# nv-tlabs/ASE

Measured on AMD Instinct MI355X. Metric: ASE PPO-update samples/sec (4096 envs x horizon 32), higher is better.
Workload: dtype f16; 1 GPU; BASELINE configs[1]: ASE agent, 4096 envs x horizon 32, obs 253 / act 31 / amp obs 1400 / latent 64, [1024,1024,512] MLPs + disc + shared-trunk encoder, minibatch 16384 (amp 4096) x 6 mini-epochs = 48 optimisation steps per update; random-init weights; precision_choice=auto without an oracle leg: the first candidate, replay=program, parallelism=single GPU

## Files before the change

### ase_amd/csrc/gemm.hip

```cpp
#include "gemm_nt.h"
#include <math.h>

namespace ase_nt {

unsigned long long* g_nt_prof = nullptr;
int g_nt_prof_clk = 0;

int nt_choice(int M, int N, int K, int es, bool b16) {
    if (N <= 64) return 0;
    const int t256 = ((M + 255) / 256) * ((N + 255) / 256);
    const bool big = N % 256 == 0 && t256 >= 192 && (t256 <= 256 || t256 % 256 == 0 || t256 >= 1024);
    if (big) {
        if (!(b16 && (K * es) % 128 == 0)) return 3;
        const int t192 = ((M + 191) / 192) * (N / 256);
        return (t256 < 256 && t192 <= 256 && t192 > t256) ? 6 : 2;
    }
    if ((K * es) % 128 != 0) return 1;
    const int t128 = ((M + 127) / 128) * ((N + 127) / 128), t64x128 = ((M + 63) / 64) * ((N + 127) / 128);
    if (t128 >= 512) return 1;
    if (t64x128 >= 512) return 4;
    return 5;
}

}

using namespace ase_nt;

extern "C" int ase_hip_debug_nt_profile(void* buf) {
    g_nt_prof = reinterpret_cast<unsigned long long*>(buf);
    return ASE_OK;
}

extern "C" int ase_hip_debug_nt_profile_clock(int shader_clock) {
    g_nt_prof_clk = shader_clock ? 1 : 0;
    return ASE_OK;
}

extern "C" int ase_hip_gemm_nt_kernel_id(int M, int N, int K, int dtype) {
    dtype &= 0xFF;
    return nt_choice(M, N, K, ase_elem_size(dtype), ase_elem_size(dtype) == 2);
}

namespace {

struct NTFused {
    const float* seed_w = nullptr; int seed_n = 0; float seed_scale = 0.f;
    void* twin = nullptr; int64_t ldtwin = 0; int twin_dtype = 0;
    double* sq_acc = nullptr; double sq_scale = 0.0; const float* sq_dyn = nullptr;
    bool any() const { return seed_w || twin || sq_acc; }
};

int gemm_nt_impl(const void* A, int64_t lda, const void* B, int64_t ldb, void* C, int64_t ldc,
                 const float* bias, const void* aux, int64_t ldaux, int aux_split, int aux_delta,
                 float* colsum, int colsum_n, void* mask_out, int64_t ldmask, int M, int N, int K, int act,
                 int aux_mode, int out_f32, float alpha, float* alpha_dev, int dtype_word, const NTFused& fu, void* stream) {
    const int dtype = dtype_word & 0xFF, ea = (dtype_word >> 8) & 0xFF, eb = (dtype_word >> 16) & 0xFF;
    const int es = ase_elem_size(dtype);
    ASE_CHECK_ARG(dtype == ASE_F32 || dtype == ASE_BF16 || dtype == ASE_F32X3 || dtype == ASE_F16 || dtype == ASE_F32H3,
                  "gemm_nt: bad dtype %d", dtype);
    ASE_CHECK_ARG(ea >= 0 && ea <= 24 && eb >= 0 && eb <= 24 && (dtype == ASE_F32H3 || (ea | eb) == 0),
                  "gemm_nt: operand scale exponents (bits 8-15 / 16-23 of dtype) are 0..24 and belong to ASE_F32H3 only");
    ASE_CHECK_ARG(A && B && (C || fu.twin) && M > 0 && N > 0 && K > 0, "gemm_nt: null/empty operand (M=%d N=%d K=%d)", M, N, K);
    if (fu.any()) {
        ASE_CHECK_ARG(dtype == ASE_F32H3 && colsum == nullptr && act <= ASE_ACT_RELU &&
                          (aux_mode == ASE_AUX_NONE || aux_mode == ASE_AUX_RELU_BITS),
                      "gemm_nt_ex: seed / twin / sum of squares belong to ASE_F32H3 launches without column sums, with no activation or "
                      "ReLU and no mask operand or a bit matrix");
        ASE_CHECK_ARG(fu.seed_w == nullptr || (fu.seed_n >= 0 && fu.seed_n <= N), "gemm_nt_ex: seed_n=%d outside [0, N]", fu.seed_n);
        ASE_CHECK_ARG(fu.twin == nullptr || ((fu.twin_dtype == ASE_F16 || fu.twin_dtype == ASE_BF16) && fu.ldtwin >= N &&
                                             ((uintptr_t)fu.twin % 8) == 0 && (fu.ldtwin * 2) % 8 == 0),
                      "gemm_nt_ex: the twin is f16 / bf16, 8-byte aligned, ldtwin >= N in whole 8-byte steps");
        ASE_CHECK_ARG(fu.sq_acc == nullptr || ((uintptr_t)fu.sq_acc % 8) == 0, "gemm_nt_ex: misaligned sq_acc");
    }
    ASE_CHECK_ARG((K * es) % 64 == 0, "gemm_nt: K=%d is not a multiple of %d elements", K, 64 / es);
    ASE_CHECK_ARG(lda >= K && ldb >= K && (ldc >= N || C == nullptr), "gemm_nt: leading dimension too small");
    ASE_CHECK_ARG(((uintptr_t)A % 16) == 0 && ((uintptr_t)B % 16) == 0 && (lda * es) % 16 == 0 && (ldb * es) % 16 == 0,
                  "gemm_nt: A/B must be 16-byte aligned with 16-byte row pitch");
    ASE_CHECK_ARG(aux_mode == ASE_AUX_NONE || aux != nullptr, "gemm_nt: aux_mode %d without aux", aux_mode);
    const bool bits = aux_mode == ASE_AUX_RELU_BITS;
    ASE_CHECK_ARG(N % 4 == 0 && ((uintptr_t)C % 16) == 0 && (ldc * (out_f32 ? 4 : es)) % 8 == 0 &&
                      (aux == nullptr || bits || (((uintptr_t)aux % 8) == 0 && (ldaux * es) % 8 == 0)),
                  "gemm_nt: C / aux must allow 8/16-byte row-vector access (N %% 4 == 0, aligned pitches)");
    ASE_CHECK_ARG(!bits || (((uintptr_t)aux % 4) == 0 && ldaux * 32 >= N), "gemm_nt: bit mask needs ldaux >= N / 32 words");
    const bool smooth = act >= ASE_ACT_SILU;
    ASE_CHECK_ARG(act >= ASE_ACT_NONE && act <= ASE_ACT_SOFTPLUS, "gemm_nt: unknown activation %d", act);
    ASE_CHECK_ARG((aux_mode & 0xFF) <= ASE_AUX_PREACT && ((aux_mode & 0xFF) == ASE_AUX_PREACT || (aux_mode >> 8) == 0) &&
                      (aux_mode >> 8) <= ASE_ACT_SOFTPLUS, "gemm_nt: bad aux_mode 0x%x", aux_mode);
// ... 54 lines not shown
```

### ase_amd/csrc/gemm_nt.h

```cpp
#pragma once
#include "common.h"
#include "act.h"
#include <type_traits>

namespace ase_nt {


__device__ __forceinline__ int xcd_remap(int bid, int nwg) {
    const int q = nwg >> 3, r = nwg & 7, xcd = bid & 7, loc = bid >> 3;
    const int base = (xcd < r) ? xcd * (q + 1) : r * (q + 1) + (xcd - r) * q;
    return base + loc;
}


template <int RB> __device__ __forceinline__ int lds_swz(int r) { return RB == 128 ? ((r >> 1) & 7) : ((r >> 2) & 3); }

typedef __attribute__((address_space(1))) const void gptr_t;
typedef __attribute__((address_space(3))) void lptr_t;

template <int N> __device__ __forceinline__ void wait_vmcnt() { asm volatile("s_waitcnt vmcnt(%0)" ::"n"(N) : "memory"); }

struct NTParams {
    const char* A; int64_t lda;
    const char* B; int64_t ldb;
// ... 70 lines not shown
template <> __device__ __forceinline__ uint32_t cvt_relu_pk16<bf16_t>(f32x2 v, float lo) {
    const f32x2 l = {lo, lo};
    return __builtin_bit_cast(uint32_t, __builtin_convertvector(__builtin_elementwise_maximum(v, l), bf16x2));
}
template <> __device__ __forceinline__ uint32_t cvt_relu_pk16<f16_t>(f32x2 v, float lo) {
    const f16_t l16 = (f16_t)__builtin_amdgcn_fmed3f(lo, -65504.f, 65504.f);
    const f16x2 hi = {(f16_t)65504.f, (f16_t)65504.f}, l = {l16, l16};
    const f16x2 c = __builtin_elementwise_maximum(__builtin_elementwise_minimum(__builtin_convertvector(v, f16x2), hi), l);
    return __builtin_bit_cast(uint32_t, c);
}

__device__ __forceinline__ uint32_t ovf_fold(uint32_t run, uint32_t packed) {
    const uint32_t mag = packed & 0x7FFF7FFFu;
    asm("v_pk_max_u16 %0, %0, %1" : "+v"(run) : "v"(mag));
    return run;
}
template <typename T> __device__ __forceinline__ bool ovf_hit(uint32_t run) {
    return (run & 0xFFFFu) >= ovf_threshold<T>() || (run >> 16) >= ovf_threshold<T>();
}

template <typename T, int AUXK, bool MASK>
__device__ __forceinline__ uint32_t rows_frag(const f32x16& c, const f32x4 (&bias)[4], uint32_t w, f32x2 al, float relu_lo, int h,
                                              uint32_t (&pk)[4][2]) {
    uint32_t mlo = 0, mhi = 0;
#pragma unroll
    for (int g = 0; g < 4; ++g)
#pragma unroll
        for (int pr = 0; pr < 2; ++pr) {
            f32x2 v = {c[g * 4 + 2 * pr], c[g * 4 + 2 * pr + 1]};
            const f32x2 b = {bias[g][2 * pr], bias[g][2 * pr + 1]};
            v = v * al + b;
            if constexpr (AUXK == 2) {
                const i32x2 keep = {(int)__builtin_amdgcn_sbfe(w, 8 * g + 2 * pr, 1), (int)__builtin_amdgcn_sbfe(w, 8 * g + 2 * pr + 1, 1)};
                v = __builtin_bit_cast(f32x2, __builtin_bit_cast(i32x2, v) & keep);
            }
            pk[g][pr] = cvt_relu_pk16<T>(v, relu_lo);
            if constexpr (MASK) {
                constexpr uint32_t INF = std::is_same<T, f16_t>::value ? 0x7C007C00u : 0x7F807F80u;
                const u16x2 one = {1, 1};
                const uint32_t d = __builtin_bit_cast(uint32_t, __builtin_bit_cast(u16x2, pk[g][pr]) - one);
                uint32_t tw;
                asm("v_pk_sub_u16 %0, %1, %2 clamp" : "=v"(tw) : "s"(INF), "v"(d));
                asm("v_pk_min_u16 %0, %0, %1" : "+v"(tw) : "s"(0x00010001u));
                const u16x2 t = __builtin_bit_cast(u16x2, tw);
                const u16x2 sh = {(unsigned short)((g & 1) * 8 + 2 * pr), (unsigned short)((g & 1) * 8 + 2 * pr + 1)};
                const uint32_t m = __builtin_bit_cast(uint32_t, t << sh);
                if (g < 2) mlo |= m; else mhi |= m;
            }
        }
    if constexpr (MASK) return ((((mlo | (mlo >> 16)) & 0xFFFFu) | ((mhi | (mhi >> 16)) << 16))) << (4 * h);
    else return 0u;
}

template <typename T, int AUXK, bool MASK, int NJ, int NI>
__device__ __forceinline__ void nt8_epilogue_rows_impl(const NTParams& p, f32x16 (&acc)[NI][NJ], int lane, int mrow0, int ncol0,
                                                       const uint32_t (&bits)[NI][NJ]) {
    const int r = lane & 31, h = lane >> 5;
    const f32x2 al = {p.alpha, p.alpha};
    const float relu_lo = (p.act == ASE_ACT_RELU) ? 0.f : -__builtin_inff();
    uint32_t ovf = 0;
    f32x4 bias[NJ][4];
#pragma unroll
    for (int j = 0; j < NJ; ++j)
#pragma unroll
        for (int g = 0; g < 4; ++g) {
            if (p.bias) bias[j][g] = *reinterpret_cast<const f32x4*>(p.bias + ncol0 + j * 32 + 8 * g + 4 * h);
            else bias[j][g] = f32x4{0.f, 0.f, 0.f, 0.f};
        }
#pragma unroll
    for (int i = 0; i < NI; ++i) {
        const int m = mrow0 + i * 32 + r;
        const bool row_ok = m < p.M;
        char* crow = p.C + (int64_t)m * p.ldc + (int64_t)ncol0 * 2 + h * 16;
        uint32_t mword[NJ];
        uint4 out[NJ][2];
#pragma unroll
        for (int j = 0; j < NJ; ++j) {
            uint32_t pk[4][2];
            mword[j] = rows_frag<T, AUXK, MASK>(acc[i][j], bias[j], AUXK == 2 ? bits[i][j] >> (4 * h) : 0u, al, relu_lo, h, pk);
#pragma unroll
            for (int g = 0; g < 4; g += 2) {
                const auto s0 = __builtin_amdgcn_permlane32_swap(pk[g][0], pk[g + 1][0], false, false);
                const auto s1 = __builtin_amdgcn_permlane32_swap(pk[g][1], pk[g + 1][1], false, false);
                out[j][g >> 1] = make_uint4(s0[0], s1[0], s0[1], s1[1]);
                ovf = ovf_fold(ovf_fold(ovf_fold(ovf_fold(ovf, s0[0]), s1[0]), s0[1]), s1[1]);
            }
        }
        if (row_ok) {
#pragma unroll
            for (int j = 0; j < NJ; ++j)
#pragma unroll
                for (int g = 0; g < 4; g += 2) *reinterpret_cast<uint4*>(crow + (j * 32 + 8 * g) * 2) = out[j][g >> 1];
        }
        if constexpr (MASK) {
#pragma unroll
            for (int jp = 0; jp < NJ; jp += 2) {
                const auto w = __builtin_amdgcn_permlane32_swap(mword[jp], mword[jp + 1], false, false);
                const uint32_t full = w[0] | w[1];
                if (row_ok) p.mask_out[(int64_t)m * p.ldmask + (ncol0 >> 5) + jp + h] = full;
            }
        }
    }
    ovf_report(p.alpha_dev, ovf_hit<T>(ovf));
}

template <typename T, int AUXK, int NJ = 2, int NI = 4>
__device__ __forceinline__ void nt8_epilogue_rows(const NTParams& p, f32x16 (&acc)[NI][NJ], int lane, int mrow0, int ncol0,
                                                  const uint32_t (&bits)[NI][NJ]) {
    if (ncol0 >= p.N) return;
    if (p.mask_out) nt8_epilogue_rows_impl<T, AUXK, true, NJ, NI>(p, acc, lane, mrow0, ncol0, bits);
    else nt8_epilogue_rows_impl<T, AUXK, false, NJ, NI>(p, acc, lane, mrow0, ncol0, bits);
}


template <int UNITS> __device__ __forceinline__ void wait_dma_units() { wait_vmcnt<2 * UNITS>(); }
__device__ __forceinline__ void wait_dma_units_rt(int units) {
    if (units >= 4) wait_vmcnt<8>();
    else if (units == 3) wait_vmcnt<6>();
    else if (units == 2) wait_vmcnt<4>();
    else if (units == 1) wait_vmcnt<2>();
    else wait_vmcnt<0>();
}
__device__ __forceinline__ void nt8_sync_in() {
    NT8_BARRIER();
    asm volatile("s_waitcnt lgkmcnt(0)" ::: "memory");
    __builtin_amdgcn_sched_barrier(0);
    __builtin_amdgcn_s_setprio(1);
}
__device__ __forceinline__ void nt8_sync_out() {
    __builtin_amdgcn_s_setprio(0);
    NT8_BARRIER();
}

#define NT_PROF_STAMP(prof, tid, slot, shader_clk)                                                              \
    do {                                                                                                        \
        if ((prof) && (tid) == 0) (prof)[slot] = (shader_clk) ? (unsigned long long)clock64() : wall_clock64(); \
    } while (0)
#define NT_PROF_CLOSE(prof, tid, slot)                         \
    do {                                                       \
        if (prof) {                                            \
            asm volatile("s_waitcnt vmcnt(0)" ::: "memory");   \
            __syncthreads();                                   \
            if ((tid) == 0) (prof)[slot] = wall_clock64();     \
        }                                                      \
    } while (0)

extern unsigned long long* g_nt_prof;
extern int g_nt_prof_clk;

int nt_choice(int M, int N, int K, int es, bool b16);

int dispatch_nt_bf16(const NTParams& p, hipStream_t s);
int dispatch_nt_f16(const NTParams& p, hipStream_t s);
int dispatch_nt_f32(const NTParams& p, hipStream_t s);
int dispatch_nt_x3(const NTParams& p, hipStream_t s);
int dispatch_nt_h3(const NTParams& p, hipStream_t s);

}
```

### ase_amd/csrc/gemm_nt_kernels.h

```cpp
#pragma once
#include "gemm_nt.h"
#include <stdlib.h>
#include <utility>

namespace {

using namespace ase_nt;

typedef uint32_t u32x4 __attribute__((ext_vector_type(4)));
template <int N, typename F, int... I> __device__ __forceinline__ void static_for_impl(F&& f, std::integer_sequence<int, I...>) {
    (f(std::integral_constant<int, I>{}), ...);
}
template <int N, typename F> __device__ __forceinline__ void static_for(F&& f) { static_for_impl<N>(f, std::make_integer_sequence<int, N>{}); }

template <typename T> struct Mma;

template <typename T> struct Mma16 {
    typedef typename V16<T>::x8 x8;
    template <int FM, int FN, int RB, bool SW = false>
    static __device__ __forceinline__ void tile(const char* sA, const char* sB, int lane, f32x16 (&acc)[FM][FN]) {
        const int r = lane & 31, h = lane >> 5, sw = lds_swz<RB>(r);
#pragma unroll
        for (int ks = 0; ks < RB / 32; ++ks) {
            x8 a[FM], b[FN];
// ... 650 lines not shown
#pragma unroll
    for (int ks = 0; ks < 4; ++ks) f[ks] = *reinterpret_cast<const i32x4*>(base + L.roff[ks]);
}

template <typename T, int KIND, bool SW, int NA = 2>
__device__ __forceinline__ void nt8_mma_issue(f32x16& c0, f32x16& c1, const i32x4 (&a0)[4], const i32x4 (&a1)[4],
                                              const i32x4 (&b)[4], const NT8Lane& L, int tile, bool live) {
#pragma unroll
    for (int ks = 0; ks < 4; ++ks) {
        if (ks == 3) NT8_BARRIER();
        c0 = nt8_mfma<T, SW>(a0[ks], b[ks], c0);
        if constexpr (NA == 2) c1 = nt8_mfma<T, SW>(a1[ks], b[ks], c1);
        if (ks == 0 || ks == 2) {
            __builtin_amdgcn_sched_barrier(0);
            if (live) nt8_piece<KIND>(L, ks >> 1, tile);
            __builtin_amdgcn_sched_barrier(0);
        }
    }
    __builtin_amdgcn_sched_barrier(0);
    __builtin_amdgcn_s_setprio(0);
    __builtin_amdgcn_sched_barrier(0);
}

template <typename T, bool TAIL, bool SW, int NI = 4>
__device__ __forceinline__ void nt8_ktile(int t, int nk, const NT8Lane& L, const char* aP, const char* bP,
                                          f32x16 (&acc)[NI][2], i32x4 (&a0)[4], i32x4 (&a1)[4], i32x4 (&b0)[4],
                                          i32x4 (&b1)[4]) {
    constexpr int RB = 128;
    const int U = 4 * nk;
    const bool l1 = !TAIL || t + 1 < nk, l2 = !TAIL || t + 2 < nk;
    nt8_read(b0, bP, L);
    nt8_read(a0, aP, L);
    nt8_read(a1, aP + 32 * RB, L);
    if (!TAIL) wait_dma_units<3>();
    else wait_dma_units_rt(min(U, 4 * t + 6) - (4 * t + 3));
    nt8_sync_in();
    nt8_mma_issue<T, 2, SW>(acc[0][0], acc[1][0], a0, a1, b0, L, t + 1, l1);
    nt8_read(b1, bP + 32 * RB, L);
    if (!TAIL) wait_dma_units<3>();
    else wait_dma_units_rt(min(U, 4 * t + 7) - (4 * t + 4));
    nt8_sync_in();
    nt8_mma_issue<T, 3, SW>(acc[0][1], acc[1][1], a0, a1, b1, L, t + 1, l1);
    nt8_read(a0, aP + 64 * RB, L);
    if constexpr (NI == 4) nt8_read(a1, aP + 96 * RB, L);
    nt8_sync_in();
    nt8_mma_issue<T, 0, SW, NI - 2>(acc[2][1], acc[NI - 1][1], a0, a1, b1, L, t + 2, l2);
    if (!TAIL) wait_dma_units<3>();
    else if (t + 1 < nk) wait_dma_units_rt(min(U, 4 * t + 9) - (4 * t + 6));
    nt8_sync_in();
    nt8_mma_issue<T, 1, SW, NI - 2>(acc[2][0], acc[NI - 1][0], a0, a1, b0, L, t + 2, l2);
}


template <typename T, bool SW, int BM = 256>
__global__ __launch_bounds__(512) void gemm_nt8_kernel(NTParams p) {
    static_assert(sizeof(T) == 2, "the phased kernel takes the 16-bit storage types");
    static_assert(BM == 256 || (BM == 192 && SW), "192-row tiles come with the row-per-lane epilogue");
    constexpr int RB = 128, BN = 256, BK = 64, WM = BM / 2, NI = WM / 32;
    constexpr int kBuf = 512 * RB;
    extern __shared__ __attribute__((aligned(16))) char smem[];
    if (p.alpha_dev) p.alpha *= *p.alpha_dev;

    const int tid = threadIdx.x, lane = tid & 63;
    const int wid = __builtin_amdgcn_readfirstlane(tid >> 6);
    const int wr = wid >> 2, wc = wid & 3;
    const int nwg = p.tiles_m * p.tiles_n;
    const int tile = xcd_remap(blockIdx.x, nwg);
    const int bm0 = (tile / p.tiles_n) * BM, bn0 = (tile % p.tiles_n) * BN;

    NT_PROF_STAMP(p.prof, tid, blockIdx.x * 4 + 0, false);
    NT8Lane L;
    {
        const int lr = lane >> 3, slot = lane & 7;
#pragma unroll
        for (int g = 0; g < 2; ++g) {
            const int ra = g * WM + wid * 8;
            const int rb = (g * 2 + (wid >> 2)) * 64 + (wid & 3) * 8;
            const int ra1 = BM == 256 ? ra + 64 : (wid >> 2) * WM + 64 + (wid & 3) * 8;
            const int rows[4] = {ra, rb, rb + 32, ra1};
#pragma unroll
            for (int kind = 0; kind < 4; ++kind) {
                const int r = rows[kind] + lr;
                const bool isB = (kind == 1 || kind == 2);
                const int64_t grow = isB ? min(bn0 + r, p.N - 1) : min(bm0 + r, p.M - 1);
                L.voff[kind][g] = (uint32_t)(grow * (isB ? p.ldb : p.lda)) + (uint32_t)((slot ^ lds_swz<RB>(r)) << 4);
                L.dst[kind][g] = (uint32_t)(uintptr_t)smem + (isB ? BM * RB : 0) + rows[kind] * RB;
            }
        }
        const int r = lane & 31, h = lane >> 5, sw = lds_swz<RB>(r);
#pragma unroll
        for (int ks = 0; ks < 4; ++ks) L.roff[ks] = r * RB + (((ks * 2 + h) ^ sw) << 4);
        L.rsA = raw_buffer(p.A);
        L.rsB = raw_buffer(p.B);
    }

    f32x16 acc[NI][2];
#pragma unroll
    for (int i = 0; i < NI; ++i)
#pragma unroll
        for (int j = 0; j < 2; ++j)
#pragma unroll
            for (int e = 0; e < 16; ++e) acc[i][j][e] = 0.f;

    AuxReg<T, 2> pre_bits[16];
    uint32_t row_bits[NI][2];
    if constexpr (!SW) {
        if (p.aux_mode == ASE_AUX_RELU_BITS) nt_aux_load<T, 4, 2, 2, 2, 2>(p, 0, lane, bm0 + wr * WM, bn0 + wc * 64, pre_bits);
    }

    const int nk = p.K / BK;
    nt8_issue<0>(L, 0);
    nt8_issue<1>(L, 0);
    nt8_issue<2>(L, 0);
    nt8_issue<3>(L, 0);
    if (nk > 1) {
        nt8_issue<0>(L, 1);
        nt8_issue<1>(L, 1);
    }
    bool mask_dma = false;
    if constexpr (SW) {
        mask_dma = p.aux_mode == ASE_AUX_RELU_BITS && bn0 + wc * 64 < p.N;
        if (mask_dma) {
            char* mlds = smem + 2 * kBuf + wid * 1024;
#pragma unroll
            for (int i = 0; i < NI; ++i) {
                const int m = bm0 + wr * WM + i * 32 + (lane & 31);
                const int ma = (m >= p.aux_split) ? m - p.aux_delta : m;
                const uint32_t* w = reinterpret_cast<const uint32_t*>(p.aux + (int64_t)min(ma, p.M - 1) * p.ldaux) +
                                    ((bn0 + wc * 64) >> 5) + (lane >> 5);
                __builtin_amdgcn_global_load_lds((gptr_t*)w, (lptr_t*)(mlds + i * 256), 4, 0, 0);
            }
        }
    }
    if (nk > 1) {
        if (mask_dma) wait_vmcnt<8 + NI>(); else wait_dma_units<4>();
    } else {
        if (mask_dma) wait_vmcnt<4 + NI>(); else wait_dma_units<2>();
    }
    NT8_BARRIER();
    NT_PROF_STAMP(p.prof, tid, blockIdx.x * 4 + 1, p.prof_clk);
    if (wr == 1) NT8_BARRIER();

    i32x4 a0[4], a1[4], b0[4], b1[4];
    const int aoff = wr * WM * RB, boff = BM * RB + wc * 64 * RB;
    int t = 0;
    for (; t + 2 < nk; ++t) {
        const char* buf = smem + (t & 1) * kBuf;
        nt8_ktile<T, false, SW, NI>(t, nk, L, buf + aoff, buf + boff, acc, a0, a1, b0, b1);
    }
    for (; t < nk; ++t) {
        const char* buf = smem + (t & 1) * kBuf;
        nt8_ktile<T, true, SW, NI>(t, nk, L, buf + aoff, buf + boff, acc, a0, a1, b0, b1);
    }
    if (wr == 0) NT8_BARRIER();
    __syncthreads();
    NT_PROF_STAMP(p.prof, tid, blockIdx.x * 4 + 2, p.prof_clk);

    float* slab = reinterpret_cast<float*>(smem) + wid * (64 * 64);
    if constexpr (SW) {
        if (p.aux_mode == ASE_AUX_RELU_BITS) {
            const uint32_t* mw = reinterpret_cast<const uint32_t*>(smem + 2 * kBuf + wid * 1024);
#pragma unroll
            for (int i = 0; i < NI; ++i) {
                row_bits[i][0] = mw[i * 64 + (lane & 31)];
                row_bits[i][1] = mw[i * 64 + 32 + (lane & 31)];
            }
            nt8_epilogue_rows<T, 2, 2, NI>(p, acc, lane, bm0 + wr * WM, bn0 + wc * 64, row_bits);
        } else nt8_epilogue_rows<T, 0, 2, NI>(p, acc, lane, bm0 + wr * WM, bn0 + wc * 64, row_bits);
    } else if constexpr (BM == 256) {
        if (p.aux_mode == ASE_AUX_RELU_BITS)
            nt_epilogue_impl<T, 4, 2, 2, 2, 2, true>(p, acc, slab, lane, bm0 + wr * 128, bn0 + wc * 64, &pre_bits);
        else
            nt_epilogue<T, 4, 2, 2, 2>(p, acc, slab, lane, bm0 + wr * 128, bn0 + wc * 64);
    }
    NT_PROF_CLOSE(p.prof, tid, blockIdx.x * 4 + 3);
}

template <typename T, bool SW = false, int BM = 256> int launch_nt8(const NTParams& p0, hipStream_t stream) {
    constexpr int lds = 2 * 512 * 128 + (SW ? 8 * 1024 : 0);
    constexpr auto kern = gemm_nt8_kernel<T, SW, BM>;
    if (const int rc = ase_dynamic_lds<kern>("gemm_nt8", lds)) return rc;
    NTParams p = p0;
    p.prof = g_nt_prof;
    p.prof_clk = g_nt_prof_clk;
    p.tiles_m = (p.M + BM - 1) / BM;
    p.tiles_n = (p.N + 255) / 256;
    ASE_LAUNCH(kern, dim3(p.tiles_m * p.tiles_n), dim3(512), lds, stream, p);
    ASE_CHECK_LAUNCH("gemm_nt8");
    return ASE_OK;
}

}
#include "gemm_nt4.h"
namespace {

inline bool rows_epi(const NTParams& p, int wave_cols) {
    return !p.out_f32 && p.N % wave_cols == 0 && p.colsum == nullptr && p.act <= ASE_ACT_RELU &&
           (p.mask_out == nullptr || p.act == ASE_ACT_RELU) &&
           (p.aux_mode == ASE_AUX_NONE || p.aux_mode == ASE_AUX_RELU_BITS);
}

template <typename T> int dispatch_nt(const NTParams& p, hipStream_t s) {
    const bool k128 = (p.K * (int)sizeof(T)) % 128 == 0;
    const bool fits32 = (int64_t)p.M * p.lda < (int64_t)0x7FFFFFFF && (int64_t)p.N * p.ldb < (int64_t)0x7FFFFFFF;
    int choice = nt_choice(p.M, p.N, p.K, (int)sizeof(T), sizeof(T) == 2);
    if ((choice == 2 || choice == 6) && !fits32) choice = 3;
    if constexpr (std::is_same<T, f32h_t>::value) {
        if (p.seed_w || p.twin || p.sq_acc) {
            switch (choice) {
                case 0: return launch_nt<T, 2, 2, 1, 1, 64, 4, 1, false, true>(p, s);
                case 2: case 3: case 6:
                    if (k128) return launch_nt<T, 4, 2, 2, 4, 128, 2, 1, false, true>(p, s);
                    return launch_nt<T, 4, 2, 2, 4, 64, 4, 1, false, true>(p, s);
                case 4: return launch_nt<T, 2, 2, 1, 2, 128, 2, 2, false, true>(p, s);
                case 5: return launch_nt<T, 2, 2, 1, 1, 128, 4, 2, false, true>(p, s);
                default:
                    if (k128) return launch_nt<T, 2, 2, 2, 2, 128, 2, 2, false, true>(p, s);
                    return launch_nt<T, 2, 2, 2, 2, 64, 4, 2, false, true>(p, s);
            }
        }
    }
    switch (choice) {
        case 0: return launch_nt<T, 2, 2, 1, 1, 64, 4>(p, s);
        case 6:
            if constexpr (sizeof(T) == 2) if (rows_epi(p, 64)) return launch_nt8<T, true, 192>(p, s);
            [[fallthrough]];
        case 2:
            if constexpr (sizeof(T) == 2) {
                if (p.M >= 65536 && rows_epi(p, 128)) return launch_nt4<T>(p, s);
                if (rows_epi(p, 64)) return launch_nt8<T, true>(p, s);
                return launch_nt8<T, false>(p, s);
            }
            [[fallthrough]];
        case 3:
            if (k128) return launch_nt<T, 4, 2, 2, 4, 128, 2>(p, s);
            return launch_nt<T, 4, 2, 2, 4, 64, 4>(p, s);
        case 4:
            if constexpr (sizeof(T) == 2) if (rows_epi(p, 64)) return launch_nt<T, 2, 2, 1, 2, 128, 2, 2, true>(p, s);
            return launch_nt<T, 2, 2, 1, 2, 128, 2, 2>(p, s);
        case 5:
            if constexpr (sizeof(T) == 2) if (rows_epi(p, 32)) return launch_nt<T, 2, 2, 1, 1, 128, 4, 2, true>(p, s);
            return launch_nt<T, 2, 2, 1, 1, 128, 4, 2>(p, s);
        default:
            if constexpr (sizeof(T) == 2) if (k128 && rows_epi(p, 64)) return launch_nt<T, 2, 2, 2, 2, 128, 2, 1, true>(p, s);
            if (k128) return launch_nt<T, 2, 2, 2, 2, 128, 2>(p, s);
            return launch_nt<T, 2, 2, 2, 2, 64, 4>(p, s);
    }
}

}
```

### ase_amd/lib.py

```python
import ctypes as C
import os

_HERE = os.path.dirname(os.path.abspath(__file__))
LIB_PATH = os.path.join(_HERE, "csrc", "libase_hip.so")

ABI_VERSION = 9
PPO_SCRATCH = 1024 * 72 + 8
PPO_SCRATCH_LS = 1024 * 136 + 8
LS_FROZEN, LS_VECTOR, LS_ROWS = 0, 1, 2
TN_SLAB = 65536 + 256
F32, BF16, F32X3, F16, F32H3 = 0, 1, 2, 3, 4
ACT_NONE, ACT_RELU, ACT_TANH, ACT_SILU, ACT_ELU, ACT_GELU, ACT_SIGMOID, ACT_SELU, ACT_SOFTPLUS = range(9)
AUX_NONE, AUX_RELU_MASK, AUX_TANH_GRAD, AUX_RELU_BITS, AUX_PREACT = 0, 1, 2, 3, 4
TASK_HEADING, TASK_LOCATION, TASK_REACH, TASK_STRIKE = range(4)
TASK_OBS_COLS = (5, 2, 3, 15)
TASK_RESET_DRAWS = (3, 2, 3, 4)
RESET_FRAME, RESET_TABLE, RESET_MOTION = range(3)
RESET_HAS_TABLE, RESET_HAS_MOTION = 1, 2
KIND_U8, KIND_I32, KIND_I64, KIND_F32 = range(4)
ROLLOUT_STORE_MAX_FIELDS, ROLLOUT_STORE_ROWS = 16, 8
INIT_DEFAULT, INIT_START, INIT_RANDOM, INIT_HYBRID = range(4)

(ACC_MASK_SUM, ACC_A_LOSS, ACC_B_LOSS, ACC_ENTROPY, ACC_CLIPPED, ACC_C_LOSS, ACC_KL, ACC_DIV, ACC_BCE_AGENT,
 ACC_BCE_DEMO, ACC_AGENT_ACC, ACC_DEMO_ACC, ACC_GP, ACC_ENC, ACC_ENC_GP, ACC_LOGIT_W2, ACC_DISC_W2, ACC_ENC_W2,
# ... 2 lines not shown
(RES_A_LOSS, RES_C_LOSS, RES_B_LOSS, RES_ENTROPY, RES_CLIP_FRAC, RES_KL, RES_DISC_LOSS, RES_DISC_GP,
 RES_DISC_LOGIT_LOSS, RES_DISC_AGENT_ACC, RES_DISC_DEMO_ACC, RES_ENC_LOSS, RES_DIV_LOSS, RES_LOSS,
 RES_MASK_SUM, RES_ENC_GP, RES_LR) = range(17)
RES_COUNT = 20

_p, _i, _i64, _f, _d = C.c_void_p, C.c_int, C.c_int64, C.c_float, C.c_double

SIGNATURES = {
    "ase_hip_gemm_nt": [_p, _i64, _p, _i64, _p, _i64, _p, _p, _i64, _i, _i, _p, _i, _p, _i64, _i, _i, _i, _i, _i, _i, _f, _p, _i, _p],
    "ase_hip_gemm_nt_ex": [_p, _i64, _p, _i64, _p, _i64, _p, _p, _i64, _i, _i, _p, _i, _p, _i64, _i, _i, _i, _i, _i, _i, _f, _p, _i,
                           _p, _i, _f, _p, _i64, _i, _p, _d, _p, _p],
    "ase_hip_gemm_tn": [_p, _i64, _p, _i64, _p, _p, _i, _i, _i, _i, _i, _i, _i, _i, _f, _p, _i, _p],
    "ase_hip_refresh_shadow": [_p, _i, _i, _p, _i64, _p, _i64, _i, _i, _i, _p],
    "ase_hip_refresh_shadow_multi": [_p, _i, _i, _p],
    "ase_hip_gather_multi": [_p, _i, _p, _i, _i, _i, _p],
    "ase_hip_rms_moments": [_p, _i64, _i, _p, _i, _i, _i, _p, _p, _p],
    "ase_hip_rms_finalize": [_p, _i, _p, _p, _i, _p, _p, _p],
    "ase_hip_rms_normalize": [_p, _i64, _i, _p, _i, _i, _i, _p, _p, _p, _i64, _p, _i64, _p, _i64, _i, _p],
    "ase_hip_rms_unnormalize": [_p, _p, _p, _i64, _p],
    "ase_hip_gather_rows": [_p, _i64, _i, _p, _i, _i, _i, _p, _i64, _i, _p],
    "ase_hip_reduce_sum": [_p, _i64, _i, _p, _i, _p],
    "ase_hip_ppo_head": [_p, _i64, _p, _i64] + [_p] * 11 + [_p, _i64, _p, _i64, _p, _p, _p, _p, _p] + [_i] * 8 + [_f] * 6 + [_p]
                        + [_i, _i64, _p, _i64, _p, _f] + [_i, _p],
    "ase_hip_disc_head": [_p, _i64, _p, _i64, _p, _p, _i, _i, _f, _f, _p, _i, _p],
    "ase_hip_enc_head": [_p, _i64, _p, _i64, _p, _i64, _p, _p, _p, _i, _i, _i, _f, _f, _p, _i, _p],
    "ase_hip_gp_seed": [_p, _i64, _p, _p, _i64, _i, _i, _f, _i, _i, _p],
    "ase_hip_gp_second": [_p, _i64, _p, _i64, _p, _i64, _p, _i64, _i, _i, _i, _i, _p],
    "ase_hip_colsum": [_p, _i64, _i, _i, _f, _p, _p],
    "ase_hip_sqnorm": [_p, _i64, _i, _i, _p, _i, _d, _p, _i, _p],
    "ase_hip_finalize_scalars": [_p, _p, _i, _i, _i, _i, _i, _i] + [_f] * 11 + [_p, _f, _p],
    "ase_hip_enc_gp_seed": [_p, _i64, _p, _i64, _p, _i64, _i, _i, _f, _i, _p],
    "ase_hip_enc_gp_back": [_p, _i64, _p, _i64, _p, _i64, _p, _i64, _p, _i, _i, _f, _p, _i, _p],
    "ase_hip_clip_scale": [_p, _i64, _p, _f, _p],
    "ase_hip_begin_step": [_p, _p, _i, _p, _i, _p, _p],
    "ase_hip_adam": [_p, _p, _p, _p, _i64, _p, _p],
    "ase_hip_axpy": [_p, _p, _i64, _f, _p],
    "ase_hip_scaler_check": [_p, _i64, _i, _p, _p],
    "ase_hip_scaler_check_multi": [_p, _i, _i, _p, _p],
    "ase_hip_scaler_fold": [_p, _p, _p],
    "ase_hip_scaler_step": [_p, _p, _p, _p, _i64, _p, _p],
    "ase_hip_disc_reward": [_p, _i64, _p, _i64, _f, _p],
    "ase_hip_enc_reward": [_p, _i64, _p, _i64, _p, _i64, _i, _f, _p],
    "ase_hip_gae": [_p, _p, _p, _p, _p, _p, _f, _f, _f, _d, _d, _p, _p, _i, _i, _p],
    "ase_hip_adv_norm": [_p, _p, _p, _p, _p, _i64, _i, _i, _p],
    "ase_hip_ring_store": [_p, _i64, _i, _p, _i, _i, _i, _p, _i64, _i64, _p],
    "ase_hip_sample_latents": [_p, _i, _i, _p, _i64, _i, _p, _i64, _i, _p],
    "ase_hip_rms_moments_multi": [_p, _p, _p, _p, _p, _p, _i, _i, _i, _p, _p],
    "ase_hip_rms_normalize_multi": [_p, _p, _p, _p, _p, _p, _p, _p, _p, _i, _i, _i, _i, _p],
    "ase_hip_rms_normalize_multi_v2": [_p, _p, _p, _p, _p, _p, _p, _p, _p, _p, _p, _i, _i, _i, _i, _p],
    "ase_hip_normalize_rows": [_p, _i64, _p, _i64, _i, _i, _p],
    "ase_hip_sample_actions": [_p, _i64, _p, _i64, _p, _p, _p, _p, _p, _p, _p, _i, _i, _i, _p],
    "ase_hip_debug_nt_profile": [_p],
    "ase_hip_debug_nt_profile_clock": [_i],
    "ase_hip_motion_state": [_p] * 6 + [_i] + [_p] * 6 + [_i, _p, _p, _i, _p, _i] + [_p] * 8,
    "ase_hip_build_amp_obs": [_p, _p, _p, _p, _p, _p, _p, _i, _i, _i, _p, _i, _i, _i, _p, _i, _i, _p],
    "ase_hip_humanoid_obs_max": [_p, _p, _p, _p, _i, _i, _i, _i, _p, _i, _p, _i64, _i, _p],
    "ase_hip_humanoid_reset": [_p, _p, _p, _p, _p, _i, _p, _p, _i, _i, _i, _f, _i, _p, _p, _p],
    "ase_hip_task_obs": [_i, _p, _p, _p, _p, _p, _i, _p, _i, _p, _i64, _i, _p],
    "ase_hip_task_reward": [_i, _p, _p, _p, _p, _p, _f, _p, _p, _i, _i, _f, _i, _p, _p],
    "ase_hip_task_reset": [_i, _p, _i, _p, _p, _p, _i, _p, _p, _i64, _i64, _p, _i64, _p, _p, _p, _p, _i64] + [_d] * 8 + [_i, _i, _p],
    "ase_hip_latent_renew": [_p, _i, _p, _i64, _p, _p, _i, _p, _i, _p, _i, _i64, _i64, _p, _i64, _p, _i64, _i, _i, _i, _p],
    "ase_hip_amp_reset": [_p] * 6 + [_i] + [_p] * 6 + [_i, _p, _i] + [_p] * 5 + [_i, _i, _p, _p, _p, _i, _p, _i64, _p, _p, _i64, _i,
                          _p, _p, _p, _p, _i, _i, _i, _f, _p, _i, _p],
    "ase_hip_amp_reset_due": [_p] * 6 + [_i] + [_p] * 6 + [_i, _p, _i] + [_p, _i] + [_p, _p, _p, _i] + [_i, _d, _i, _d, _d, _i]
                             + [_p, _i] + [_p] * 4 + [_p] * 5 + [_p, _i64, _p, _p, _i64, _i] + [_p] * 4 + [_i, _i, _i, _f, _p, _i, _p],
    "ase_hip_amp_demo_fetch": [_p] * 6 + [_i] + [_p] * 4 + [_i, _p, _p, _i, _p, _i] + [_p] * 4 + [_i, _p, _p] + [_i, _i, _f, _f, _i, _i]
                              + [_p, _i64, _i, _i, _p, _p],
    "ase_hip_rollout_store": [_p, _i, _p, _f, _f, _p, _i64, _p, _i, _p, _i64, _p, _p, _i, _p, _i64, _p, _p, _p, _i, _p, _i64, _p,
                              _i, _i, _p, _i, _p],
    "ase_hip_hrl_latent": [_p, _i64, _p, _i64, _p, _i64, _i, _i, _i, _p],
    "ase_hip_hrl_llc_action": [_p, _i64, _p, _p, _p, _i64, _i, _i, _i, _p],
    "ase_hip_hrl_accum": [_p, _p, _i, _p, _i, _p, _i64, _f, _p, _i64, _i, _i, _i, _p, _p, _p, _p, _i, _p],
    "ase_hip_clip_frames": [_p] * 6 + [_i] + [_p] * 4 + [_i, _i, _p, _p, _i] + [_p] * 7,
    "ase_hip_gemm_nt_kernel_id": [_i, _i, _i, _i],
    "ase_hip_gemm_tn_kernel_id": [_i, _i, _i, _i, _i, _i64, _i64, _i],
    "ase_hip_apply_multi": [_p, _i, _p, _p, _i, _p],
    "ase_hip_apply_multi_v2": [_p, _i, _p, _p, _p, _i, _p],
    "ase_hip_gemm_tn_grouped_plan": [_p, _i, _i, _p, _i, _p, _p, _i, _p],
    "ase_hip_prog_create": [_p],
    "ase_hip_prog_destroy": [_p],
    "ase_hip_prog_begin": [_p],
    "ase_hip_prog_end": [_p],
    "ase_hip_prog_size": [_p],
    "ase_hip_prog_launch": [_p],
    "ase_hip_prog_host": [_p, _p],
    "ase_hip_mark": [_p, _p],
    "ase_hip_wait": [_p, _i],
    "ase_hip_memset": [_p, _i, _i64, _p],
    "ase_hip_memcpy": [_p, _p, _i64, _p],
    "ase_hip_gemm_tn_grouped": [_p, _p, _i, _p, _i, _p, _p, _i, _p],
}


class AseHipError(RuntimeError):
    pass


def rollout_store_ws(n_envs):
    return 3 * ((int(n_envs) + ROLLOUT_STORE_ROWS - 1) // ROLLOUT_STORE_ROWS)


def load():
    import torch
    if not os.path.exists(LIB_PATH):
        raise AseHipError(
            f"{LIB_PATH} is missing: build it with `python -c 'import __graft_entry__ as g; g.build()'` "
# ... 27 lines not shown
```

### include/ase_hip.h

```cpp
#ifndef ASE_HIP_H
#define ASE_HIP_H

#include <stdint.h>

#ifdef __cplusplus
extern "C" {
#endif

#define ASE_HIP_ABI_VERSION 9

enum { ASE_F32 = 0, ASE_BF16 = 1, ASE_F32X3 = 2 ,
       ASE_F32H3 = 4 ,
       ASE_F16 = 3  };
enum { ASE_ACT_NONE = 0, ASE_ACT_RELU = 1, ASE_ACT_TANH = 2, ASE_ACT_SILU = 3, ASE_ACT_ELU = 4, ASE_ACT_GELU = 5,
       ASE_ACT_SIGMOID = 6, ASE_ACT_SELU = 7, ASE_ACT_SOFTPLUS = 8 };
enum { ASE_AUX_NONE = 0, ASE_AUX_RELU_MASK = 1, ASE_AUX_TANH_GRAD = 2, ASE_AUX_RELU_BITS = 3 ,
       ASE_AUX_PREACT = 4  };
enum { ASE_OK = 0, ASE_EINVAL = -1, ASE_ELAUNCH = -2, ASE_EUNSUPPORTED = -3 };

int ase_hip_abi_version(void);
const char* ase_hip_last_error(void);

int ase_hip_gemm_nt_kernel_id(int M, int N, int K, int dtype);

int ase_hip_debug_nt_profile(void* buf);
int ase_hip_debug_nt_profile_clock(int shader_clock);


int ase_hip_gemm_nt(const void* A, int64_t lda, const void* B, int64_t ldb, void* C, int64_t ldc,
                    const float* bias, const void* aux, int64_t ldaux, int aux_split, int aux_delta,
                    float* colsum, int colsum_n, void* mask_out, int64_t ldmask, int M, int N, int K, int act,
                    int aux_mode, int out_f32, float alpha, float* alpha_dev, int dtype, void* stream);

int ase_hip_gemm_nt_ex(const void* A, int64_t lda, const void* B, int64_t ldb, void* C, int64_t ldc,
                       const float* bias, const void* aux, int64_t ldaux, int aux_split, int aux_delta,
                       float* colsum, int colsum_n, void* mask_out, int64_t ldmask, int M, int N, int K, int act,
                       int aux_mode, int out_f32, float alpha, float* alpha_dev, int dtype,
                       const float* seed_w, int seed_n, float seed_scale, void* twin, int64_t ldtwin, int twin_dtype,
                       double* sq_acc, double sq_scale, const float* sq_dyn, void* stream);

int ase_hip_gemm_tn(const void* A, int64_t lda, const void* B, int64_t ldb, float* G, float* gbias,
                    int bias_rows, int M, int N, int K, int n_real, int k_real, int split_src, int split_dst,
                    float alpha, const float* alpha_dev, int dtype, void* stream);

int ase_hip_gemm_tn_kernel_id(int M, int N, int K, int n_real, int bias_rows, int64_t lda, int64_t ldb, int dtype);

#define ASE_TN_SLAB (65536 + 256)
int ase_hip_gemm_tn_grouped_plan(int64_t* problems, int n_problems, int target_wg, int32_t* work, int max_work,
                                 int* n_work, int32_t* red, int max_red, int* n_red);
int ase_hip_gemm_tn_grouped(const int64_t* problems, const int32_t* work, int n_work, const int32_t* red, int n_red,
                            float* workspace, const float* alpha_dev, int dtype, void* stream);

int ase_hip_refresh_shadow(const float* W, int n_real, int k_real, void* Ws, int64_t ldws,
                           void* Wts, int64_t ldwts, int split_src, int split_dst, int dtype,
                           void* stream);

int ase_hip_refresh_shadow_multi(const int64_t* desc, int n_layers, int dtype, void* stream);


int ase_hip_rms_moments(const float* src, int64_t ld_src, int D, const int32_t* idx, int remap_h,
                        int remap_n, int M, const double* state, double* sums, void* stream);

int ase_hip_rms_moments_multi(const float* const* srcs, const int64_t* ld_srcs, const int32_t* const* idxs,
                              const int* remap_h, const int* remap_n, double* const* sums, int n_streams, int D, int M,
                              const double* state, void* stream);
int ase_hip_rms_normalize_multi(const float* const* srcs, const int64_t* ld_srcs, const int32_t* const* idxs,
                                const int* remap_h, const int* remap_n, const float* const* means,
                                const float* const* stds, void* const* outs, const int64_t* ld_outs, int n_streams, int D,
                                int M, int dtype, void* stream);
int ase_hip_rms_normalize_multi_v2(const float* const* srcs, const int64_t* ld_srcs, const int32_t* const* idxs,
                                   const int* remap_h, const int* remap_n, const float* const* means,
                                   const float* const* stds, void* const* outs, const int64_t* ld_outs,
                                   float* const* outs32, const int64_t* ld_outs32, int n_streams, int D, int M, int dtype,
                                   void* stream);

int ase_hip_rms_finalize(double* state, int D, const double* sums, const int32_t* counts ,
                         int n_streams, float* mean_out, float* std_out, void* stream);

int ase_hip_rms_normalize(const float* src, int64_t ld_src, int D, const int32_t* idx, int remap_h,
// ... 267 lines not shown
```

Baseline: 1.837 million samples/s.

## Add persistent two-tile NT GEMM kernel overlapping next tile's loads with epilogue

Adds a persistent variant of the 256-column phased NT GEMM kernel. Each workgroup loops over tiles with a grid capped at the CU count, and issues the next tile's prologue loads before running the current tile's register epilogue, so global-memory latency overlaps with output stores. By default it is used when the row-per-lane path is chosen, the launch has no seed/twin/sum-of-squares fusion, and there are more tiles than CUs. A debug knob can force it or set the grid size. The cost is extra register pressure from holding bias and mask bits across the prefetch, plus a few kernel specialisations for the epilogue variants.

```diff
diff --git a/ase_amd/csrc/gemm.hip b/ase_amd/csrc/gemm.hip
--- a/ase_amd/csrc/gemm.hip
+++ b/ase_amd/csrc/gemm.hip
@@ -5,6 +5,17 @@
 
 unsigned long long* g_nt_prof = nullptr;
 int g_nt_prof_clk = 0;
+int g_nt_persist = -1;
+
+int nt_cu_count() {
+    static const int cus = [] {
+        int dev = 0, n = 0;
+        if (hipGetDevice(&dev) != hipSuccess || hipDeviceGetAttribute(&n, hipDeviceAttributeMultiprocessorCount, dev) != hipSuccess) n = 0;
+        return n;
+    }();
+    if (cus <= 0) ase_set_error("gemm_nt: the device's compute unit count is not available");
+    return cus;
+}
 
 int nt_choice(int M, int N, int K, int es, bool b16) {
     if (N <= 64) return 0;
@@ -33,6 +44,11 @@
 
 extern "C" int ase_hip_debug_nt_profile_clock(int shader_clock) {
     g_nt_prof_clk = shader_clock ? 1 : 0;
+    return ASE_OK;
+}
+
+extern "C" int ase_hip_debug_nt_persistent(int max_workgroups) {
+    g_nt_persist = max_workgroups < 0 ? -1 : max_workgroups;
     return ASE_OK;
 }
 
diff --git a/ase_amd/csrc/gemm_nt.h b/ase_amd/csrc/gemm_nt.h
--- a/ase_amd/csrc/gemm_nt.h
+++ b/ase_amd/csrc/gemm_nt.h
@@ -146,21 +146,25 @@
     else return 0u;
 }
 
+template <int NJ>
+__device__ __forceinline__ void nt8_rows_bias(const NTParams& p, int lane, int ncol0, f32x4 (&bias)[NJ][4]) {
+    const int h = lane >> 5;
+#pragma unroll
+    for (int j = 0; j < NJ; ++j)
+#pragma unroll
+        for (int g = 0; g < 4; ++g) {
+            if (p.bias) bias[j][g] = *reinterpret_cast<const f32x4*>(p.bias + ncol0 + j * 32 + 8 * g + 4 * h);
+            else bias[j][g] = f32x4{0.f, 0.f, 0.f, 0.f};
+        }
+}
+
 template <typename T, int AUXK, bool MASK, int NJ, int NI>
-__device__ __forceinline__ void nt8_epilogue_rows_impl(const NTParams& p, f32x16 (&acc)[NI][NJ], int lane, int mrow0, int ncol0,
-                                                       const uint32_t (&bits)[NI][NJ]) {
+__device__ __forceinline__ void nt8_epilogue_rows_body(const NTParams& p, f32x16 (&acc)[NI][NJ], int lane, int mrow0, int ncol0,
+                                                       const uint32_t (&bits)[NI][NJ], const f32x4 (&bias)[NJ][4]) {
     const int r = lane & 31, h = lane >> 5;
     const f32x2 al = {p.alpha, p.alpha};
     const float relu_lo = (p.act == ASE_ACT_RELU) ? 0.f : -__builtin_inff();
     uint32_t ovf = 0;
-    f32x4 bias[NJ][4];
-#pragma unroll
-    for (int j = 0; j < NJ; ++j)
-#pragma unroll
-        for (int g = 0; g < 4; ++g) {
-            if (p.bias) bias[j][g] = *reinterpret_cast<const f32x4*>(p.bias + ncol0 + j * 32 + 8 * g + 4 * h);
-            else bias[j][g] = f32x4{0.f, 0.f, 0.f, 0.f};
-        }
 #pragma unroll
     for (int i = 0; i < NI; ++i) {
         const int m = mrow0 + i * 32 + r;
@@ -196,6 +200,14 @@
         }
     }
     ovf_report(p.alpha_dev, ovf_hit<T>(ovf));
+}
+
+template <typename T, int AUXK, bool MASK, int NJ, int NI>
+__device__ __forceinline__ void nt8_epilogue_rows_impl(const NTParams& p, f32x16 (&acc)[NI][NJ], int lane, int mrow0, int ncol0,
+                                                       const uint32_t (&bits)[NI][NJ]) {
+    f32x4 bias[NJ][4];
+    nt8_rows_bias<NJ>(p, lane, ncol0, bias);
+    nt8_epilogue_rows_body<T, AUXK, MASK, NJ, NI>(p, acc, lane, mrow0, ncol0, bits, bias);
 }
 
 template <typename T, int AUXK, int NJ = 2, int NI = 4>
@@ -241,6 +253,8 @@
 
 extern unsigned long long* g_nt_prof;
 extern int g_nt_prof_clk;
+extern int g_nt_persist;
+int nt_cu_count();
 
 int nt_choice(int M, int N, int K, int es, bool b16);
 
diff --git a/ase_amd/csrc/gemm_nt_kernels.h b/ase_amd/csrc/gemm_nt_kernels.h
--- a/ase_amd/csrc/gemm_nt_kernels.h
+++ b/ase_amd/csrc/gemm_nt_kernels.h
@@ -726,63 +726,36 @@
 }
 
 
-template <typename T, bool SW, int BM = 256>
-__global__ __launch_bounds__(512) void gemm_nt8_kernel(NTParams p) {
-    static_assert(sizeof(T) == 2, "the phased kernel takes the 16-bit storage types");
-    static_assert(BM == 256 || (BM == 192 && SW), "192-row tiles come with the row-per-lane epilogue");
-    constexpr int RB = 128, BN = 256, BK = 64, WM = BM / 2, NI = WM / 32;
-    constexpr int kBuf = 512 * RB;
-    extern __shared__ __attribute__((aligned(16))) char smem[];
-    if (p.alpha_dev) p.alpha *= *p.alpha_dev;
-
-    const int tid = threadIdx.x, lane = tid & 63;
-    const int wid = __builtin_amdgcn_readfirstlane(tid >> 6);
-    const int wr = wid >> 2, wc = wid & 3;
-    const int nwg = p.tiles_m * p.tiles_n;
-    const int tile = xcd_remap(blockIdx.x, nwg);
-    const int bm0 = (tile / p.tiles_n) * BM, bn0 = (tile % p.tiles_n) * BN;
-
-    NT_PROF_STAMP(p.prof, tid, blockIdx.x * 4 + 0, false);
-    NT8Lane L;
-    {
-        const int lr = lane >> 3, slot = lane & 7;
-#pragma unroll
-        for (int g = 0; g < 2; ++g) {
-            const int ra = g * WM + wid * 8;
-            const int rb = (g * 2 + (wid >> 2)) * 64 + (wid & 3) * 8;
-            const int ra1 = BM == 256 ? ra + 64 : (wid >> 2) * WM + 64 + (wid & 3) * 8;
-            const int rows[4] = {ra, rb, rb + 32, ra1};
-#pragma unroll
-            for (int kind = 0; kind < 4; ++kind) {
-                const int r = rows[kind] + lr;
-                const bool isB = (kind == 1 || kind == 2);
-                const int64_t grow = isB ? min(bn0 + r, p.N - 1) : min(bm0 + r, p.M - 1);
-                L.voff[kind][g] = (uint32_t)(grow * (isB ? p.ldb : p.lda)) + (uint32_t)((slot ^ lds_swz<RB>(r)) << 4);
-                L.dst[kind][g] = (uint32_t)(uintptr_t)smem + (isB ? BM * RB : 0) + rows[kind] * RB;
-            }
-        }
-        const int r = lane & 31, h = lane >> 5, sw = lds_swz<RB>(r);
-#pragma unroll
-        for (int ks = 0; ks < 4; ++ks) L.roff[ks] = r * RB + (((ks * 2 + h) ^ sw) << 4);
-        L.rsA = raw_buffer(p.A);
-        L.rsB = raw_buffer(p.B);
-    }
-
-    f32x16 acc[NI][2];
-#pragma unroll
-    for (int i = 0; i < NI; ++i)
-#pragma unroll
-        for (int j = 0; j < 2; ++j)
-#pragma unroll
-            for (int e = 0; e < 16; ++e) acc[i][j][e] = 0.f;
-
-    AuxReg<T, 2> pre_bits[16];
-    uint32_t row_bits[NI][2];
-    if constexpr (!SW) {
-        if (p.aux_mode == ASE_AUX_RELU_BITS) nt_aux_load<T, 4, 2, 2, 2, 2>(p, 0, lane, bm0 + wr * WM, bn0 + wc * 64, pre_bits);
-    }
-
-    const int nk = p.K / BK;
+template <int BM>
+__device__ __forceinline__ void nt8_lane_setup(NT8Lane& L, const NTParams& p, const char* smem, int bm0, int bn0, int lane, int wid) {
+    constexpr int RB = 128, WM = BM / 2;
+    const int lr = lane >> 3, slot = lane & 7;
+#pragma unroll
+    for (int g = 0; g < 2; ++g) {
+        const int ra = g * WM + wid * 8;
+        const int rb = (g * 2 + (wid >> 2)) * 64 + (wid & 3) * 8;
+        const int ra1 = BM == 256 ? ra + 64 : (wid >> 2) * WM + 64 + (wid & 3) * 8;
+        const int rows[4] = {ra, rb, rb + 32, ra1};
+#pragma unroll
+        for (int kind = 0; kind < 4; ++kind) {
+            const int r = rows[kind] + lr;
+            const bool isB = (kind == 1 || kind == 2);
+            const int64_t grow = isB ? min(bn0 + r, p.N - 1) : min(bm0 + r, p.M - 1);
+            L.voff[kind][g] = (uint32_t)(grow * (isB ? p.ldb : p.lda)) + (uint32_t)((slot ^ lds_swz<RB>(r)) << 4);
+            L.dst[kind][g] = (uint32_t)(uintptr_t)smem + (isB ? BM * RB : 0) + rows[kind] * RB;
+        }
+    }
+    const int r = lane & 31, h = lane >> 5, sw = lds_swz<RB>(r);
+#pragma unroll
+    for (int ks = 0; ks < 4; ++ks) L.roff[ks] = r * RB + (((ks * 2 + h) ^ sw) << 4);
+    L.rsA = raw_buffer(p.A);
+    L.rsB = raw_buffer(p.B);
+}
+
+template <bool SW, int BM>
+__device__ __forceinline__ bool nt8_prologue_issue(const NT8Lane& L, const NTParams& p, char* smem, int nk, int bm0, int bn0,
+                                                   int lane, int wid) {
+    constexpr int WM = BM / 2, NI = WM / 32, kBuf = 512 * 128;
     nt8_issue<0>(L, 0);
     nt8_issue<1>(L, 0);
     nt8_issue<2>(L, 0);
@@ -793,6 +766,7 @@
     }
     bool mask_dma = false;
     if constexpr (SW) {
+        const int wr = wid >> 2, wc = wid & 3;
         mask_dma = p.aux_mode == ASE_AUX_RELU_BITS && bn0 + wc * 64 < p.N;
         if (mask_dma) {
             char* mlds = smem + 2 * kBuf + wid * 1024;
@@ -806,17 +780,78 @@
             }
         }
     }
+    return mask_dma;
+}
+
+template <typename T, bool SW, int BM, bool PERSIST, int EPI>
+__device__ __forceinline__ void nt8_kernel_body(NTParams p) {
+    static_assert(sizeof(T) == 2, "the phased kernel takes the 16-bit storage types");
+    static_assert(BM == 256 || (BM == 192 && SW), "192-row tiles come with the row-per-lane epilogue");
+    static_assert(!PERSIST || SW, "the two-tile form stores from registers: row-per-lane epilogue only");
+    constexpr int RB = 128, BN = 256, BK = 64, WM = BM / 2, NI = WM / 32;
+    constexpr int kBuf = 512 * RB;
+    extern __shared__ __attribute__((aligned(16))) char smem[];
+    if (p.alpha_dev) p.alpha *= *p.alpha_dev;
+
+    const int tid = threadIdx.x, lane = tid & 63;
+    const int wid = __builtin_amdgcn_readfirstlane(tid >> 6);
+    const int wr = wid >> 2, wc = wid & 3;
+    const int nwg = p.tiles_m * p.tiles_n;
+    int index = blockIdx.x;
+    const int tile = xcd_remap(index, nwg);
+    int bm0 = (tile / p.tiles_n) * BM, bn0 = (tile % p.tiles_n) * BN;
+
+    NT_PROF_STAMP(p.prof, tid, index * 4 + 0, false);
+    NT8Lane L;
+    f32x16 acc[NI][2];
+    if constexpr (!PERSIST) {
+    nt8_lane_setup<BM>(L, p, smem, bm0, bn0, lane, wid);
+
+#pragma unroll
+    for (int i = 0; i < NI; ++i)
+#pragma unroll
+        for (int j = 0; j < 2; ++j)
+#pragma unroll
+            for (int e = 0; e < 16; ++e) acc[i][j][e] = 0.f;
+    }
+
+    AuxReg<T, 2> pre_bits[16];
+    uint32_t row_bits[NI][2];
+    if constexpr (!SW) {
+        if (p.aux_mode == ASE_AUX_RELU_BITS) nt_aux_load<T, 4, 2, 2, 2, 2>(p, 0, lane, bm0 + wr * WM, bn0 + wc * 64, pre_bits);
+    }
+
+    const int nk = p.K / BK;
+    bool mask_dma;
+    if constexpr (PERSIST) {
+        NT8Lane L0;
+        nt8_lane_setup<BM>(L0, p, smem, bm0, bn0, lane, wid);
+        mask_dma = nt8_prologue_issue<SW, BM>(L0, p, smem, nk, bm0, bn0, lane, wid);
+    } else mask_dma = nt8_prologue_issue<SW, BM>(L, p, smem, nk, bm0, bn0, lane, wid);
+    const int aoff = wr * WM * RB, boff = BM * RB + wc * 64 * RB;
+#pragma nounroll
+    for (;;) {
+    if constexpr (PERSIST) {
+        int l1 = lane;
+        asm volatile("" : "+v"(l1));
+        nt8_lane_setup<BM>(L, p, smem, bm0, bn0, l1, wid);
+#pragma unroll
+        for (int i = 0; i < NI; ++i)
+#pragma unroll
+            for (int j = 0; j < 2; ++j)
+#pragma unroll
+                for (int e = 0; e < 16; ++e) acc[i][j][e] = 0.f;
+    }
     if (nk > 1) {
         if (mask_dma) wait_vmcnt<8 + NI>(); else wait_dma_units<4>();
     } else {
         if (mask_dma) wait_vmcnt<4 + NI>(); else wait_dma_units<2>();
     }
     NT8_BARRIER();
-    NT_PROF_STAMP(p.prof, tid, blockIdx.x * 4 + 1, p.prof_clk);
+    NT_PROF_STAMP(p.prof, tid, index * 4 + 1, p.prof_clk);
     if (wr == 1) NT8_BARRIER();
 
     i32x4 a0[4], a1[4], b0[4], b1[4];
-    const int aoff = wr * WM * RB, boff = BM * RB + wc * 64 * RB;
     int t = 0;
     for (; t + 2 < nk; ++t) {
         const char* buf = smem + (t & 1) * kBuf;
@@ -828,7 +863,54 @@
     }
     if (wr == 0) NT8_BARRIER();
     __syncthreads();
-    NT_PROF_STAMP(p.prof, tid, blockIdx.x * 4 + 2, p.prof_clk);
+    NT_PROF_STAMP(p.prof, tid, index * 4 + 2, p.prof_clk);
+
+    if constexpr (PERSIST) {
+        const int mrow0 = bm0 + wr * WM, ncol0 = bn0 + wc * 64;
+        constexpr bool bits = (EPI & 1) != 0;
+        const bool cols = ncol0 < p.N;
+        int ln = lane;
+        asm volatile("" : "+v"(ln));
+        if (bits) {
+            const uint32_t* mw = reinterpret_cast<const uint32_t*>(smem + 2 * kBuf + wid * 1024);
+#pragma unroll
+            for (int i = 0; i < NI; ++i) {
+                row_bits[i][0] = mw[i * 64 + (ln & 31)];
+                row_bits[i][1] = mw[i * 64 + 32 + (ln & 31)];
+            }
+#pragma unroll
+            for (int i = 0; i < NI; ++i) asm volatile("" : "+v"(row_bits[i][0]), "+v"(row_bits[i][1]));
+        }
+        f32x4 bias[2][4];
+        if (cols) {
+            nt8_rows_bias<2>(p, ln, ncol0, bias);
+#pragma unroll
+            for (int j = 0; j < 2; ++j)
+#pragma unroll
+                for (int g = 0; g < 4; ++g) asm volatile("" : "+v"(bias[j][g]));
+        }
+        const int next = index + (int)gridDim.x;
+        const bool more = next < nwg;
+        if (more) {
+            const int tn = xcd_remap(next, nwg);
+            bm0 = (tn / p.tiles_n) * BM;
+            bn0 = (tn % p.tiles_n) * BN;
+            NT_PROF_STAMP(p.prof, tid, next * 4 + 0, false);
+            NT8Lane Ln;
+            nt8_lane_setup<BM>(Ln, p, smem, bm0, bn0, ln, wid);
+            mask_dma = nt8_prologue_issue<SW, BM>(Ln, p, smem, nk, bm0, bn0, ln, wid);
+        }
+        if (cols) {
+            nt8_epilogue_rows_body<T, bits ? 2 : 0, (EPI & 2) != 0, 2, NI>(p, acc, ln, mrow0, ncol0, row_bits, bias);
+        }
+        if (!more) {
+            NT_PROF_CLOSE(p.prof, tid, index * 4 + 3);
+            return;
+        }
+        NT_PROF_STAMP(p.prof, tid, index * 4 + 3, false);
+        index = next;
+        continue;
+    }
 
     float* slab = reinterpret_cast<float*>(smem) + wid * (64 * 64);
     if constexpr (SW) {
@@ -847,21 +929,58 @@
         else
             nt_epilogue<T, 4, 2, 2, 2>(p, acc, slab, lane, bm0 + wr * 128, bn0 + wc * 64);
     }
-    NT_PROF_CLOSE(p.prof, tid, blockIdx.x * 4 + 3);
-}
-
-template <typename T, bool SW = false, int BM = 256> int launch_nt8(const NTParams& p0, hipStream_t stream) {
+    NT_PROF_CLOSE(p.prof, tid, index * 4 + 3);
+    return;
+    }
+}
+
+template <typename T, bool SW, int BM = 256>
+__global__ __launch_bounds__(512) void gemm_nt8_kernel(NTParams p) {
+    nt8_kernel_body<T, SW, BM, false, 0>(p);
+}
+
+template <typename T, int BM, int EPI>
+__global__ __launch_bounds__(512) void gemm_nt8p_kernel(NTParams p) {
+    nt8_kernel_body<T, true, BM, true, EPI>(p);
+}
+
+template <typename T, bool SW, int BM, bool PERSIST, int EPI> constexpr auto nt8_kernel_of() {
+    if constexpr (PERSIST) return gemm_nt8p_kernel<T, BM, EPI>;
+    else return gemm_nt8_kernel<T, SW, BM>;
+}
+
+template <typename T, bool SW, int BM, bool PERSIST, int EPI = 0> int launch_nt8_grid(const NTParams& p0, int grid, hipStream_t stream) {
     constexpr int lds = 2 * 512 * 128 + (SW ? 8 * 1024 : 0);
-    constexpr auto kern = gemm_nt8_kernel<T, SW, BM>;
+    constexpr auto kern = nt8_kernel_of<T, SW, BM, PERSIST, EPI>();
     if (const int rc = ase_dynamic_lds<kern>("gemm_nt8", lds)) return rc;
     NTParams p = p0;
     p.prof = g_nt_prof;
     p.prof_clk = g_nt_prof_clk;
     p.tiles_m = (p.M + BM - 1) / BM;
     p.tiles_n = (p.N + 255) / 256;
-    ASE_LAUNCH(kern, dim3(p.tiles_m * p.tiles_n), dim3(512), lds, stream, p);
+    const int tiles = p.tiles_m * p.tiles_n;
+    ASE_LAUNCH(kern, dim3(PERSIST ? min(grid, tiles) : tiles), dim3(512), lds, stream, p);
     ASE_CHECK_LAUNCH("gemm_nt8");
     return ASE_OK;
+}
+
+template <typename T, bool SW = false, int BM = 256> int launch_nt8(const NTParams& p, hipStream_t stream) {
+    if constexpr (SW) {
+        const int tiles = ((p.M + BM - 1) / BM) * ((p.N + 255) / 256);
+        const int cus = nt_cu_count();
+        if (cus <= 0) return ASE_ELAUNCH;
+        const bool fused = p.seed_w || p.twin || p.sq_acc;
+        if (!fused && (g_nt_persist >= 0 || tiles > cus)) {
+            const int grid = g_nt_persist > 0 ? g_nt_persist : cus;
+            switch ((p.aux_mode == ASE_AUX_RELU_BITS ? 1 : 0) | (p.mask_out ? 2 : 0)) {
+                case 0: return launch_nt8_grid<T, true, BM, true, 0>(p, grid, stream);
+                case 1: return launch_nt8_grid<T, true, BM, true, 1>(p, grid, stream);
+                case 2: return launch_nt8_grid<T, true, BM, true, 2>(p, grid, stream);
+                default: return launch_nt8_grid<T, true, BM, true, 3>(p, grid, stream);
+            }
+        }
+    }
+    return launch_nt8_grid<T, SW, BM, false>(p, 0, stream);
 }
 
 }
@@ -894,6 +1013,12 @@
             }
         }
     }
+    if constexpr (sizeof(T) == 2) {
+        if (g_nt_persist >= 0 && k128 && fits32 && rows_epi(p, 64)) {
+            if (choice == 6 || (choice != 2 && p.M % 192 == 0 && p.M % 256 != 0)) return launch_nt8<T, true, 192>(p, s);
+            return launch_nt8<T, true>(p, s);
+        }
+    }
     switch (choice) {
         case 0: return launch_nt<T, 2, 2, 1, 1, 64, 4>(p, s);
         case 6:
diff --git a/ase_amd/lib.py b/ase_amd/lib.py
--- a/ase_amd/lib.py
+++ b/ase_amd/lib.py
@@ -78,6 +78,7 @@
     "ase_hip_sample_actions": [_p, _i64, _p, _i64, _p, _p, _p, _p, _p, _p, _p, _i, _i, _i, _p],
     "ase_hip_debug_nt_profile": [_p],
     "ase_hip_debug_nt_profile_clock": [_i],
+    "ase_hip_debug_nt_persistent": [_i],
     "ase_hip_motion_state": [_p] * 6 + [_i] + [_p] * 6 + [_i, _p, _p, _i, _p, _i] + [_p] * 8,
     "ase_hip_build_amp_obs": [_p, _p, _p, _p, _p, _p, _p, _i, _i, _i, _p, _i, _i, _i, _p, _i, _i, _p],
     "ase_hip_humanoid_obs_max": [_p, _p, _p, _p, _i, _i, _i, _i, _p, _i, _p, _i64, _i, _p],
diff --git a/include/ase_hip.h b/include/ase_hip.h
--- a/include/ase_hip.h
+++ b/include/ase_hip.h
@@ -25,6 +25,7 @@
 
 int ase_hip_debug_nt_profile(void* buf);
 int ase_hip_debug_nt_profile_clock(int shader_clock);
+int ase_hip_debug_nt_persistent(int max_workgroups);
 
 
 int ase_hip_gemm_nt(const void* A, int64_t lda, const void* B, int64_t ldb, void* C, int64_t ldc,
```

After: 1.802 million samples/s. 1.9% lower.
